# youmi-zym/TemporalStereo

Hardware: AMD Instinct MI355X
Metric: stereo pairs/sec, FlyingThings3D 540x960 D=192 (aggregation hot path) (higher is better)
Workload: dtype f32

## Files before the change

include/ts_hip.h:

```cpp
#ifndef TS_HIP_H
#define TS_HIP_H

#include <stddef.h>
#include <stdint.h>

#ifdef __cplusplus
extern "C" {
#endif

#define TS_OK 0
#define TS_ERR_NULL (-1)
#define TS_ERR_SHAPE (-2)
#define TS_ERR_UNSUPPORTED (-3)
#define TS_ERR_ALIGN (-4)

int ts_version(void);
const char* ts_last_error_string(void);

size_t ts_block_cost_workspace_bytes(int B, int C, int H, int W, int D, int scales);

int ts_block_cost_int_fwd(const float* left, const float* right, float* out, void* workspace,
                          int B, int C, int H, int W, int D, int scales, void* stream);

int ts_block_cost_sampled_fwd(const float* left, const float* right, const float* disp, float* out,
// ... 271 lines not shown
int ts_conv_wgrad_take(void* host_table, size_t capacity_bytes, int* n, int* total_blocks);
int ts_conv_wgrad_finish_many(const void* table, int n, int total_blocks, void* stream);
int ts_conv_set_chunk_cap(int cap);
int ts_conv3d_hw_fwd(const float* x, const float* w_t, const float* scale, const float* shift, float* y,
                     int B, int Cin, int Cout, int D, int H, int W, int stride, int dilation,
                     int transposed, int act, float act_param,
                     long long in_bstride, long long in_cstride, long long out_bstride,
                     long long out_cstride, const float* addend, long long addend_bstride,
                     void* workspace, size_t workspace_bytes, void* stream);
size_t ts_conv3d_hw_warp_workspace_bytes(int B, int Cout, int D, int H, int W);
int ts_conv3d_hw_warp_fwd(const float* corr, const float* w_t, const float* scale, const float* shift, float* y,
                          const float* q, const float* disp, const float* base,
                          int B, int Cc, int Cout, int D, int H, int W, int dilation, int act, float act_param,
                          long long in_bstride, long long in_cstride, long long out_bstride, long long out_cstride,
                          long long base_bstride, void* workspace, size_t workspace_bytes, void* stream);

size_t ts_conv3d_hw_workspace_bytes(int B, int Cin, int Cout, int D, int H, int W, int stride, int transposed);
int ts_conv3d_hw_x6_supported(int Cin, int Cout, int W, int stride, int dilation, int transposed);
size_t ts_conv3d_hw_x6_weight_bytes(int Cin, int Cout);
size_t ts_conv3d_hw_x6_workspace_bytes(int B, int Cin, int Cout, int D, int H, int W);
int ts_conv3d_hw_x6_weight_split(const float* w_t, void* w6, int Cin, int Cout, void* stream);
int ts_conv3d_hw_x6_weight_split_from(const float* w, void* w6, int Cin, int Cout, long long stride_ci, long long stride_co,
                                      long long stride_t, int flip, void* stream);
int ts_conv3d_hw_x6_fwd(const float* x, const void* w6, const float* scale, const float* shift, float* y,
                        int B, int Cin, int Cout, int D, int H, int W, int dilation, int act, float act_param,
                        long long in_bstride, long long in_cstride, long long out_bstride, long long out_cstride,
                        const float* addend, long long addend_bstride, void* workspace, size_t workspace_bytes, void* stream);
typedef struct ts_peer_ctx {
  void* region[8];
  int rank, world;
// ... 118 lines not shown
```

temporalstereo_amd/_lib.py:

```python
import ctypes
import os
import threading

_HERE = os.path.dirname(os.path.abspath(__file__))
LIB_PATH = os.path.join(_HERE, "libts_hip.so")

_lock = threading.Lock()
_lib = None

c_f32p = ctypes.c_void_p
c_ptr = ctypes.c_void_p
c_int = ctypes.c_int
c_size = ctypes.c_size_t
c_float = ctypes.c_float

SIGNATURES = {
    "ts_version": (c_int, []),
    "ts_last_error_string": (ctypes.c_char_p, []),
    "ts_block_cost_workspace_bytes": (c_size, [c_int] * 6),
    "ts_block_cost_int_fwd": (c_int, [c_f32p, c_f32p, c_f32p, c_ptr] + [c_int] * 6 + [c_ptr]),
    "ts_block_cost_sampled_fwd": (c_int, [c_f32p, c_f32p, c_f32p, c_f32p, c_ptr] + [c_int] * 6 + [c_ptr]),
    "ts_block_cost_sampled_warped_fwd": (c_int, [c_f32p, c_f32p, c_f32p, c_f32p, c_ptr] + [c_int] * 6 + [c_ptr]),
    "ts_block_cost_sampled_corr_fwd": (c_int, [c_f32p, c_f32p, c_f32p, c_f32p, c_ptr] + [c_int] * 6 + [c_ptr]),
    "ts_block_cost_corr_split_supported": (c_int, [c_int] * 2),
    "ts_block_cost_sampled_corr_split_fwd": (c_int, [c_f32p] * 6 + [c_ptr] + [c_int] * 7 + [ctypes.c_longlong] * 4 + [c_ptr]),
    "ts_conv3d_hw_split_supported": (c_int, [c_int] * 10),
    "ts_conv3d_hw_split_fwd": (c_int, [c_f32p] * 6 + [c_int] * 11 + [c_float] + [ctypes.c_longlong] * 6 +
                               [c_f32p, ctypes.c_longlong, c_ptr, c_size, c_ptr]),
    "ts_conv3d_d_split_supported": (c_int, [c_int] * 2),
    "ts_conv3d_d_split_fwd": (c_int, [c_f32p] * 6 + [c_int] * 13 + [c_float] + [ctypes.c_longlong] * 6 + [c_ptr]),
    "ts_conv3d_hw_x6_split_supported": (c_int, [c_int] * 5),
    "ts_conv3d_hw_x6_split_fwd": (c_int, [c_f32p, c_f32p, c_ptr, c_f32p, c_f32p, c_f32p] + [c_int] * 9 + [c_float] + [ctypes.c_longlong] * 6 +
                                  [c_f32p, ctypes.c_longlong, c_ptr, c_size, c_ptr]),
    "ts_conv3d_hw_warp_workspace_bytes": (c_size, [c_int] * 5),
    "ts_conv3d_hw_warp_fwd": (c_int, [c_f32p] * 8 + [c_int] * 8 + [c_float] + [ctypes.c_longlong] * 5 + [c_ptr, c_size, c_ptr]),
    "ts_cat_fms_fwd": (c_int, [c_f32p] * 4 + [c_int] * 5 + [c_ptr]),
    "ts_inverse_warp_3d_fwd": (c_int, [c_f32p] * 3 + [c_int] * 5 + [c_ptr]),
    "ts_dif_fms_workspace_bytes": (c_size, []),
    "ts_dif_fms_fwd": (c_int, [c_f32p] * 4 + [c_ptr] + [c_int] * 5 + [c_ptr]),
    "ts_correlation_fwd": (c_int, [c_f32p] * 3 + [c_int] * 7 + [c_ptr]),
    "ts_correlation_bwd": (c_int, [c_f32p] * 6 + [c_int] * 7 + [c_ptr]),
    "ts_block_cost_bwd_workspace_bytes": (c_size, [c_int] * 6),
    "ts_block_cost_int_bwd": (c_int, [c_f32p] * 5 + [c_ptr] + [c_int] * 6 + [c_ptr]),
    "ts_block_cost_sampled_bwd": (c_int, [c_f32p] * 7 + [c_ptr] + [c_int] * 6 + [c_ptr]),
    "ts_block_cost_sampled_warped_bwd": (c_int, [c_f32p] * 7 + [c_ptr] + [c_int] * 6 + [c_ptr]),
    "ts_calib_stream": (c_int, [c_int, c_ptr, c_ptr, c_size, c_ptr]),
    "ts_candidates_in_range_fwd": (c_int, [c_f32p] * 3 + [c_int] * 5 + [c_ptr]),
    "ts_candidates_in_range_bwd": (c_int, [c_f32p] * 5 + [c_int] * 5 + [c_ptr]),
    "ts_offset_head_fwd": (c_int, [c_f32p] * 2 + [ctypes.c_longlong, c_float, c_ptr]),
    "ts_offset_head_bwd": (c_int, [c_f32p] * 3 + [ctypes.c_longlong, c_float, c_ptr]),
# ... 122 lines not shown
    "ts_pool3d5_avgmax_bwd": (c_int, [c_f32p] * 4 + [c_int] * 5 + [c_ptr]),
    "ts_merge_candidates_bwd": (c_int, [c_f32p] * 5 + [c_int] * 5 + [c_ptr]),
    "ts_copy_rows_fwd": (c_int, [c_f32p] * 2 + [ctypes.c_longlong] * 4 + [c_ptr]),
    "ts_plan_create": (c_ptr, []),
    "ts_plan_destroy": (None, [c_ptr]),
    "ts_plan_length": (c_int, [c_ptr]),
    "ts_plan_add_call": (c_int, [c_ptr, ctypes.c_char_p, ctypes.POINTER(ctypes.c_ulonglong), c_int]),
    "ts_plan_run": (c_int, [c_ptr]),
    "ts_stream_fork": (c_int, [c_ptr, c_ptr]),
    "ts_event_record": (c_int, [c_int, c_ptr]),
    "ts_event_wait": (c_int, [c_int, c_ptr]),
}

_QUERIES = frozenset(n for n in SIGNATURES if n.endswith("_bytes") or n.startswith("ts_plan_") or
                     n.endswith("_split_supported") or
                     n in ("ts_version", "ts_last_error_string", "ts_conv_cout_pad", "ts_conv3d_hw_x6_supported", "ts_conv3d_hw_x6s_supported", "ts_peer_max_floats", "ts_peer_max_ranks",
                           "ts_peer_alloc", "ts_peer_open", "ts_peer_close", "ts_peer_free", "ts_peer_status", "ts_peer_status_async",
                           "ts_peer_set_timeout_ms", "ts_peer_reset", "ts_bn_set_small_elems",
                           "ts_conv_wgrad_defer", "ts_conv_wgrad_pending", "ts_conv_wgrad_take"))


def lib():
    rec = getattr(_tls, "recorder", None)
    if rec is not None:
        return rec.proxy
    return _real_lib()


def _real_lib():
    global _lib
    if _lib is None:
# ... 123 lines not shown
```

temporalstereo_amd/aggregation/native.py:

```python
import os
import time

import torch
import torch.nn as nn

from .. import _lib
from .. import functional as TF

ACT_NONE, ACT_SILU, ACT_RELU, ACT_TANH_OFFSET, ACT_HEAD_PAIR = 0, 1, 2, 3, 4


def _stream():
    return _lib.current_stream_handle()


_PAR = {"on": False, "aux": None, "kinds": frozenset(__import__("os").environ.get("TS_BRANCHES", "hourglass").split(","))}


def _aux_stream():
    return _PAR["aux"]


_STAGE_CAP = int(os.environ.get("TS_STAGE_CHUNK_CAP", "8"))

# ... 428 lines not shown
    rc = _lib.lib().ts_conv3d_d_fwd(_lib.ptr(x), _lib.ptr(f.w), _lib.ptr(f.scale), _lib.ptr(f.shift), _lib.ptr(out),
                                    B, Cin, f.cout, Din, H, W, k, stride, dilation, padding, int(transposed),
                                    f.act if act is None else act, float(act_param), ib, ic, ob, oc, _stream())
    _lib.check(rc, "ts_conv3d_d_fwd")
    return out


FUSED_K1 = os.environ.get("TS_FUSED_K1", "1") != "0"
SPLIT_INPUT = os.environ.get("TS_SPLIT_INPUT", "1") != "0"


def block_cost_corr(left, right, disp, scales):
    return TF.block_cost_corr(left, right, disp, scales)


def conv_hw_warp(corr, f, q, disp, base, dilation=1):
    B, Cc, D, H, W = corr.shape
    assert Cc == f.cin, (Cc, f.cin)
    out = torch.empty((B, f.cout, D, H, W), device=corr.device, dtype=torch.float32)
    ib, ic = _strides5(corr)
    ob, oc = _strides5(out)
    wsb = TF._q("ts_conv3d_hw_warp_workspace_bytes", B, f.cout, D, H, W)
    ws = torch.empty(wsb, device=corr.device, dtype=torch.uint8)
    rc = _lib.lib().ts_conv3d_hw_warp_fwd(_lib.ptr(corr), _lib.ptr(f.w), _lib.ptr(f.scale), _lib.ptr(f.shift), _lib.ptr(out),
                                          _lib.ptr(q), _lib.ptr(disp), _lib.ptr(base), B, Cc, f.cout, D, H, W, dilation, f.act, 0.0,
                                          ib, ic, ob, oc, base.stride(0) if base is not None else 0, _lib.ptr(ws), wsb, _stream())
    _lib.check(rc, "ts_conv3d_hw_warp_fwd")
    return out


def resize_add_act(a, add, size, act=ACT_SILU):
    B, C, Da, Ha, Wa = a.shape
    D, H, W = size
    out = torch.empty((B, C, D, H, W), device=a.device, dtype=torch.float32)
    ab, ac = _strides5(a)
    bb, bc = _strides5(add) if add is not None else (0, 0)
    ob, oc = _strides5(out)
    rc = _lib.lib().ts_resize3d_add_act_fwd(_lib.ptr(a), _lib.ptr(add), _lib.ptr(out), B, C, Da, Ha, Wa, D, H, W, act,
                                            ab, ac, bb, bc, ob, oc, _stream())
    _lib.check(rc, "ts_resize3d_add_act_fwd")
    return out

# ... 188 lines not shown
        self.init0, self.hg, self.init2 = SepConv(mod.init3d[0]), Hourglass(mod.init3d[1]), SepConv(mod.init3d[2])
        self.heads = Heads(mod.pred_heads)

    def init3d(self, raw, addend=None):
        return self.init2(self.hg(self.init0(raw, addend=addend)))

    def split_reference_half(self):
        if self.init0.stride != 1 or self.init0.transposed:
            raise NotImplementedError("first aggregation layer is not a stride-1 conv over [left | warped | corr]")
        self.init0_left, self.init0.f0, self.init0_corr, self.init0_q = split_sampled_first_layer(self.init0.f0, self.scales)

    def left_term(self, left):
        return conv_hw(left.unsqueeze(2), self.init0_left, 1, self.init0.dil)

    def right_term(self, right):
        return conv_d(right.unsqueeze(2), self.init0_q, 1).squeeze(2)

    def first_layer_fused(self, left, right, ds, lterm, rterm):
        corr = block_cost_corr(left, right, ds, self.scales)
        i0 = self.init0
        y = conv_hw_warp(corr, self.init0_corr, rterm, ds, lterm.squeeze(2) if lterm.dim() == 5 else lterm, i0.dil)
        return conv_d(y, i0.f1, i0.k, i0.stride, i0.dil, i0.pad_d, i0.transposed)

    def init3d_from(self, first):
        return self.init2(self.hg(first))

    def feature_terms(self, left, right):
        return self.left_term(left), (self.right_term(right) if FUSED_K1 else None)


class _MergingLevel(_LevelBase):
# ... 144 lines not shown
            return
        rc = _lib.lib().ts_deconv2d_k4s2_fwd(_lib.ptr(x), _lib.ptr(f.w), _lib.ptr(f.scale), _lib.ptr(f.shift), _lib.ptr(out),
                                             B, Cin, f.cout, H, W, f.act, out_bstride, _stream())
        _lib.check(rc, "ts_deconv2d_k4s2_fwd")

    def unet_features(self, left, right, left_image, right_image):
        both, lterm, st = self.unet_encode(left, right, left_image, right_image)
        return both, (self.unet_decode(st), lterm)

    def split_input_ok(self, B, Cf, H, W):
        L = _lib.lib()
        if self.in_planes != Cf or self.enc[3].cout != Cf:
            return False
        hw = lambda f, dil: L.ts_conv3d_hw_split_supported(B, 2 * Cf, Cf, f.cout, 1, H, W, 1, dil, 0)
        return bool(L.ts_block_cost_corr_split_supported(2 * Cf, Cf) and hw(self.init0_left, self.init0.dil) and hw(self.fuse[0], 1) and
                    (not FUSED_K1 or L.ts_conv3d_d_split_supported(2 * Cf, Cf)) and
                    (not X6 or not L.ts_conv3d_hw_x6_supported(2 * Cf, self.fuse[0].cout, W, 1, 1, 0) or
                     L.ts_conv3d_hw_x6_split_supported(2 * Cf, Cf, self.fuse[0].cout, W, 1)))

    def unet_encode(self, left, right, left_image, right_image):
        B, Cf, H, W = left.shape
        if SPLIT_INPUT and FUSED_K1 and self.split_input_ok(B, Cf, H, W):
            left, right = _lib.contiguous(left), _lib.contiguous(right)
            both = SplitBoth(left, right, torch.empty((2 * B, Cf, H, W), device=left.device, dtype=torch.float32))
            lcat, rcat = both.pair()
        else:
            both = torch.empty((2 * B, 2 * Cf, H, W), device=left.device, dtype=torch.float32)
            lcat, rcat = both[:B], both[B:]
            copy_rows(left, lcat[:, :Cf]); copy_rows(right, rcat[:, :Cf])
        C32, C2 = self.deconv4.cout, self.enc[1].cout
        cat2 = torch.empty((B, C32 + C2, 2 * H, 2 * W), device=left.device, dtype=torch.float32)
# ... 262 lines not shown
```

temporalstereo_amd/csrc/conv3d.hip:

```cpp
#include <cstdlib>
#include <mutex>
#include <type_traits>
#include <vector>

#include "conv_common.hpp"
#include "conv_x6p.hpp"
#include "warp.hpp"

namespace {




template <int MODE, int KT, int ST, int DL, int TP = 256>
struct Geom {
  static constexpr int NTR = (MODE == MODE_D) ? KT : 1;
  static constexpr int TRW = (TP == 64) ? 4 : 8, TCW = (TP == 64) ? 16 : 32;
  static constexpr int in_rows = (MODE == MODE_HW) ? (TRW - 1) * ST + 2 * DL + 1 : ((MODE == MODE_HWT) ? ((KT == 16) ? TRW + 2 : TRW + 1) : 1);
  static constexpr int in_cols = (MODE == MODE_HW) ? (TCW - 1) * ST + 2 * DL + 1 : ((MODE == MODE_HWT) ? ((KT == 16) ? TCW + 2 : TCW + 1) : TP);
  static constexpr int pitch = (MODE == MODE_D) ? TP : (in_cols | 1);
  static constexpr int RQ_HW = (in_rows * in_cols + 255) / 256;
  static constexpr int chan_raw = (MODE == MODE_D) ? NTR * TP : in_rows * pitch;
  static constexpr int pad0 = (16 - (chan_raw & 31)) & 31;
  static constexpr int chan_elems = chan_raw + (pad0 ? pad0 : 32);
// ... 1227 lines not shown
  else if (dilation == 2) rc = launch_ig<MODE_HW, 9, 1, 2>(x, w_t, scale, shift, y, p, B, tiles, D, st);
  else rc = launch_ig<MODE_HW, 9, 1, 1>(x, w_t, scale, shift, y, p, B, tiles, D, st);
  if (rc || !split) return rc;
  const long long plane = static_cast<long long>(D) * p.Ho * p.Wo;
  TS_REQUIRE(static_cast<long long>(B) * Cout <= 65535 && plane < (1ll << 31), TS_ERR_UNSUPPORTED, "conv3d_hw: split-K finish grid too large");
  long long blocks = (plane + 255) / 256;
  const long long cap = (4096 + static_cast<long long>(B) * Cout - 1) / (static_cast<long long>(B) * Cout);
  if (blocks > cap) blocks = cap;
  hipLaunchKernelGGL(conv_splitk_finish, dim3(static_cast<unsigned>(blocks), static_cast<unsigned>(B * Cout)), dim3(256), 0, st, p.partial, scale, shift, y,
                     B, Cout, plane, ksplit, act, act_param, out_bstride, out_cstride, addend, addend_bstride,
                     static_cast<long long>(p.Ho) * p.Wo);
  return ts::launched("conv_splitk_finish");
}


template <int DL>
__global__ void __launch_bounds__(256)
warp_gather_kernel(const float* __restrict__ q, const float* __restrict__ disp, const float* __restrict__ base,
                   float* __restrict__ out, int Cout, int D, int H, int W, long long base_bstride) {
  const int cogs = (Cout + 7) / 8;
  unsigned lin = blockIdx.x;
  {
    const unsigned per = gridDim.x / 8;
    if (lin < per * 8) lin = (lin % 8) * per + lin / 8;
  }
  const int d = static_cast<int>(lin % D);
  const unsigned nblk = (static_cast<unsigned>(H) * W + 255u) / 256u;
  const unsigned blk = (lin / D) % nblk;
  const int bc = static_cast<int>(lin / (static_cast<unsigned>(D) * nblk));
  const int cog = bc % cogs, b = bc / cogs;
  const unsigned HW = static_cast<unsigned>(H) * W;
// ... 8 lines not shown
#pragma unroll
  for (int t = 0; t < 9; ++t) {
    const int qy = y + (t / 3 - 1) * DL, qx = x + (t % 3 - 1) * DL;
    in[t] = live && qy >= 0 && qy < H && qx >= 0 && qx < W;
    dv[t] = __uint_as_float(__builtin_amdgcn_raw_buffer_load_b32(drs, in[t] ? (static_cast<unsigned>(qy) * W + qx) * 4u : kOOB, 0, 0));
  }
  float acc[8];
#pragma unroll
  for (int c = 0; c < 8; ++c) {
    const int co = min(cog * 8 + c, Cout - 1);
    acc[c] = (base && live) ? base[static_cast<size_t>(b) * base_bstride + static_cast<size_t>(co) * HW + pix] : 0.f;
  }
#pragma unroll
  for (int t = 0; t < 9; ++t) {
    const int qy = y + (t / 3 - 1) * DL, qx = x + (t % 3 - 1) * DL;
    const float ix = ts::source_position(qx, dv[t], W, Wm1);
    const float fl = floorf(ix);
    const float f = ix - fl;
    const int xi = static_cast<int>(fl);
    const int xb = min(max(xi, 0), W - 2);
    float wa = 0.f, wb = 0.f;
    if (xi >= 0 && xi <= W - 2) { wa = 1.f - f; wb = f; }
    else if (xi == -1) wa = f;
    else if (xi == W - 1) wb = 1.f - f;
    if (!in[t]) { wa = 0.f; wb = 0.f; }
    const unsigned voff = in[t] ? (static_cast<unsigned>(qy) * W + xb) * 4u : 0u;
#pragma unroll
    for (int c = 0; c < 8; ++c) {
      const unsigned plane = static_cast<unsigned>(t * Cout + min(cog * 8 + c, Cout - 1));
      const u32x2 v = __builtin_bit_cast(u32x2, __builtin_amdgcn_raw_buffer_load_b64(qrs, voff, plane * HW * 4u, 0));
      acc[c] += wa * __uint_as_float(v.x) + wb * __uint_as_float(v.y);
    }
  }
  if (live) {
#pragma unroll
    for (int c = 0; c < 8; ++c) {
      const int co = cog * 8 + c;
      if (co < Cout) out[((static_cast<size_t>(b) * Cout + co) * D + d) * HW + pix] = acc[c];
    }
  }
}

template <int CB, int DL, int TR = 8>
int launch_x6(const float* x, const void* w6, const float* scale, const float* shift, float* y, const IG& p, dim3 grid, hipStream_t st) {
  constexpr int NPIXP = (TR + 2 * DL) * 40;
  constexpr size_t lds = (static_cast<size_t>(3) * 2 * NPIXP + 3 * X6_SLOTS * 2 * CB * 16 + 1) * 16;
  static_assert(lds <= 80 * 1024, "ig_conv_x6_kernel: two workgroups per CU");
// ... 221 lines not shown
                                      int transposed, int act, float act_param,
                                      long long in_bstride, long long in_cstride, long long in2_bstride, long long in2_cstride,
                                      long long out_bstride, long long out_cstride, const float* addend, long long addend_bstride,
                                      void* workspace, size_t workspace_bytes, void* stream) {
  const SplitIn sp{x2, Csplit, in2_bstride, in2_cstride};
  return conv_hw_impl(x, w_t, scale, shift, y, B, Cin, Cout, D, H, W, stride, dilation, transposed, act, act_param,
                      in_bstride, in_cstride, out_bstride, out_cstride, addend, addend_bstride, workspace, workspace_bytes,
                      0, 0, stream, 0, 0, &sp);
}

extern "C" size_t ts_conv3d_hw_warp_workspace_bytes(int B, int Cout, int D, int H, int W) {
  if (B <= 0 || Cout <= 0 || D <= 0 || H <= 0 || W <= 0) return 0;
  return ts::round_up(static_cast<size_t>(B) * Cout * D * H * W * sizeof(float), 256);
}

extern "C" int ts_conv3d_hw_warp_fwd(const float* corr, const float* w_t, const float* scale, const float* shift, float* y,
                                     const float* q, const float* disp, const float* base,
                                     int B, int Cc, int Cout, int D, int H, int W, int dilation, int act, float act_param,
                                     long long in_bstride, long long in_cstride, long long out_bstride, long long out_cstride,
                                     long long base_bstride, void* workspace, size_t workspace_bytes, void* stream) {
  TS_REQUIRE(B > 0 && Cc > 0 && Cout > 0 && D > 0 && H > 0 && W >= 2, TS_ERR_SHAPE, "conv3d_hw_warp: bad size");
  TS_REQUIRE(dilation == 1 || dilation == 2, TS_ERR_UNSUPPORTED, "conv3d_hw_warp: dilation must be 1 or 2");
  TS_REQUIRE(D <= 65535 && static_cast<long long>(B) * ((Cout + 7) / 8) <= 65535, TS_ERR_UNSUPPORTED, "conv3d_hw_warp: grid too large");
  TS_REQUIRE_PTR(corr); TS_REQUIRE_PTR(w_t); TS_REQUIRE_PTR(y); TS_REQUIRE_PTR(q); TS_REQUIRE_PTR(disp); TS_REQUIRE_PTR(workspace);
  TS_REQUIRE(workspace_bytes >= ts_conv3d_hw_warp_workspace_bytes(B, Cout, D, H, W), TS_ERR_SHAPE, "conv3d_hw_warp: workspace too small");
  TS_REQUIRE(9ull * Cout * H * W * 4ull < 0x7fffffffull, TS_ERR_UNSUPPORTED, "conv3d_hw_warp: a batch element of q spans 2 GiB or more");
  hipStream_t st = ts::as_stream(stream);
  float* T = reinterpret_cast<float*>(workspace);
  const long long HW = static_cast<long long>(H) * W;
  const long long wgs = ((HW + 255) / 256) * D * B * ((Cout + 7) / 8);
  TS_REQUIRE(wgs < (1ll << 31), TS_ERR_UNSUPPORTED, "conv3d_hw_warp: grid too large");
  const dim3 grid(static_cast<unsigned>(wgs));
  if (dilation == 1) hipLaunchKernelGGL(warp_gather_kernel<1>, grid, dim3(256), 0, st, q, disp, base, T, Cout, D, H, W, base_bstride);
  else hipLaunchKernelGGL(warp_gather_kernel<2>, grid, dim3(256), 0, st, q, disp, base, T, Cout, D, H, W, base_bstride);
  if (int rc = ts::launched("warp_gather_kernel")) return rc;
  return conv_hw_impl(corr, w_t, scale, shift, y, B, Cc, Cout, D, H, W, 1, dilation, 0, act, act_param, in_bstride, in_cstride,
                      out_bstride, out_cstride, T, static_cast<long long>(Cout) * D * HW, nullptr, 0, 0, 0, stream,
                      static_cast<long long>(D) * HW, HW);
}

extern "C" int ts_conv3d_hw_bwd_data(const float* dy, const float* w_b, float* dx, int B, int Cin, int Cout, int D, int H,
                                     int W, int stride, int dilation, int transposed, long long dy_bstride,
                                     long long dy_cstride, long long dx_bstride, long long dx_cstride, void* stream) {
  TS_REQUIRE(B > 0 && Cin > 0 && Cout > 0 && D > 0 && H > 0 && W > 0, TS_ERR_SHAPE, "conv3d_hw_bwd_data: non-positive size");
  TS_REQUIRE(stride == 1 || stride == 2, TS_ERR_UNSUPPORTED, "conv3d_hw_bwd_data: stride must be 1 or 2");
  if (transposed)
    return conv_hw_impl(dy, w_b, nullptr, nullptr, dx, B, Cout, Cin, D, 2 * H, 2 * W, 2, 1, 0, ACT_NONE, 0.f, dy_bstride,
                        dy_cstride, dx_bstride, dx_cstride, nullptr, 0, nullptr, 0, 0, 0, stream);
  const int Ho = (H - 1) / stride + 1, Wo = (W - 1) / stride + 1;
  if (stride == 2)
    return conv_hw_impl(dy, w_b, nullptr, nullptr, dx, B, Cout, Cin, D, Ho, Wo, 2, 1, 1, ACT_NONE, 0.f, dy_bstride,
                        dy_cstride, dx_bstride, dx_cstride, nullptr, 0, nullptr, 0, H, W, stream);
  return conv_hw_impl(dy, w_b, nullptr, nullptr, dx, B, Cout, Cin, D, Ho, Wo, 1, dilation, 0, ACT_NONE, 0.f, dy_bstride,
// ... 228 lines not shown
```

temporalstereo_amd/csrc/plan.hip:

```cpp
#include <cstdint>
#include <cstring>
#include <mutex>
#include <string>
#include <utility>
#include <vector>

#include "ts_common.hpp"

namespace {

constexpr int kMaxWords = 32;

template <class T>
T unpack(unsigned long long w) {
  static_assert(sizeof(T) <= sizeof(unsigned long long), "argument wider than a plan word");
  T v;
  std::memcpy(&v, &w, sizeof(T));
  return v;
}

template <class... A, size_t... I>
int call_with(int (*f)(A...), const unsigned long long* w, std::index_sequence<I...>) {
  return f(unpack<A>(w[I])...);
}
// ... 57 lines not shown
    TS_PLAN_OP(ts_deconv2d_k4s2_weight_to_conv3), TS_PLAN_OP(ts_deconv2d_k4s2_wgrad_from_conv3),
    TS_PLAN_OP(ts_clip_rmsprop_step),       TS_PLAN_OP(ts_bn_sync_merge),
    TS_PLAN_OP(ts_bn_fold_many),
    TS_PLAN_OP(ts_conv_weight_layout_many2), TS_PLAN_OP(ts_conv_wgrad_finish_many), TS_PLAN_OP(ts_channel_sum_fwd),
    TS_PLAN_OP(ts_block_cost_sampled_warped_bwd),
    TS_PLAN_OP(ts_frames_prepare_fwd),      TS_PLAN_OP(ts_intrinsics_pyramid_fwd),  TS_PLAN_OP(ts_disp_u16_decode_fwd),
    TS_PLAN_OP(ts_frames_augment_fwd),      TS_PLAN_OP(ts_disp_u16_window_fwd),
    TS_PLAN_OP(ts_block_cost_sampled_corr_split_fwd), TS_PLAN_OP(ts_conv3d_hw_split_fwd),
    TS_PLAN_OP(ts_conv3d_d_split_fwd),      TS_PLAN_OP(ts_conv3d_hw_x6_split_fwd),
    TS_PLAN_OP(ts_inverse_warp_fwd),        TS_PLAN_OP(ts_inverse_warp_bwd),
    TS_PLAN_OP(ts_raft_corr_pyramid_fwd),   TS_PLAN_OP(ts_raft_corr_lookup_fwd),
    TS_PLAN_OP(ts_raft_corr_lookup_bwd),    TS_PLAN_OP(ts_raft_corr_pyramid_bwd),
    TS_PLAN_OP(ts_flow_corr_pyramid_fwd),   TS_PLAN_OP(ts_flow_corr_lookup_fwd),
    TS_PLAN_OP(ts_flow_corr_lookup_bwd),    TS_PLAN_OP(ts_flow_corr_pyramid_bwd),
    TS_PLAN_OP(ts_flow_metrics_fwd),        TS_PLAN_OP(ts_flow_render_fwd),         TS_PLAN_OP(ts_flow_u16_decode_fwd),
};

struct Call {
  const Entry* op;
  unsigned long long w[kMaxWords];
};

__global__ void __launch_bounds__(256)
copy_rows_kernel(const float* __restrict__ src, float* __restrict__ dst, long long rows, long long row_elems,
                 long long src_pitch, long long dst_pitch) {
  const long long n = rows * row_elems;
  for (long long i = static_cast<long long>(blockIdx.x) * blockDim.x + threadIdx.x; i < n;
       i += static_cast<long long>(gridDim.x) * blockDim.x) {
    const long long r = i / row_elems, c = i - r * row_elems;
    dst[r * dst_pitch + c] = src[r * src_pitch + c];
// ... 149 lines not shown
```

temporalstereo_amd/csrc/ts_common.hpp:

```cpp
#pragma once
#include <hip/hip_runtime.h>

#include <cstdarg>
#include <cstdint>
#include <cstdio>
#include <cstdlib>
#include <type_traits>

#include "../../include/ts_hip.h"

#define TS_ABI_VERSION 17

namespace ts {

char* err_buf();
int fail(int code, const char* fmt, ...);

inline hipStream_t as_stream(void* s) { return reinterpret_cast<hipStream_t>(s); }

inline bool aligned16(const void* p) { return (reinterpret_cast<uintptr_t>(p) & 15u) == 0; }

inline size_t round_up(size_t v, size_t a) { return (v + a - 1) / a * a; }

inline int launched(const char* what) {
  hipError_t e = hipGetLastError();
  if (e != hipSuccess) return fail(static_cast<int>(e), "%s: %s", what, hipGetErrorString(e));
// ... 31 lines not shown
```

Measured before the change: 1563.

## Add MFMA 1x1 conv producing tap-major q layout and vectorized warp gather

Adds a new MFMA-based 1x1 convolution kernel that writes the right-term q tensor in a channel-interleaved (groups of 8) layout, and a q8 variant of the warp gather kernel that reads 8 channels per tap with 128-bit buffer loads instead of eight strided 64-bit loads. The right_term path switches to this kernel by default when shapes allow. The aim is to cut the gather's memory transactions and replace the generic conv_d path for the pointwise projection. It adds a new layout wrapper type, so other consumers of q must handle it or call planar().

```diff
diff --git a/include/ts_hip.h b/include/ts_hip.h
--- a/include/ts_hip.h
+++ b/include/ts_hip.h
@@ -309,6 +309,15 @@
                           int B, int Cc, int Cout, int D, int H, int W, int dilation, int act, float act_param,
                           long long in_bstride, long long in_cstride, long long out_bstride, long long out_cstride,
                           long long base_bstride, void* workspace, size_t workspace_bytes, void* stream);
+int ts_conv1x1_q_supported(int Cin, int Csplit, int N);
+int ts_conv1x1_q_fwd(const float* x, const float* x2, const float* w_t, float* q, int B, int Cin, int Csplit, int N, int H, int W,
+                     long long in_bstride, long long in_cstride, long long in2_bstride, long long in2_cstride,
+                     int pixel_run, void* stream);
+int ts_conv3d_hw_warp_q8_fwd(const float* corr, const float* w_t, const float* scale, const float* shift, float* y,
+                             const float* q, const float* disp, const float* base,
+                             int B, int Cc, int Cout, int D, int H, int W, int dilation, int act, float act_param,
+                             long long in_bstride, long long in_cstride, long long out_bstride, long long out_cstride,
+                             long long base_bstride, void* workspace, size_t workspace_bytes, void* stream);
 
 size_t ts_conv3d_hw_workspace_bytes(int B, int Cin, int Cout, int D, int H, int W, int stride, int transposed);
 int ts_conv3d_hw_x6_supported(int Cin, int Cout, int W, int stride, int dilation, int transposed);
diff --git a/temporalstereo_amd/_lib.py b/temporalstereo_amd/_lib.py
--- a/temporalstereo_amd/_lib.py
+++ b/temporalstereo_amd/_lib.py
@@ -34,6 +34,9 @@
                                   [c_f32p, ctypes.c_longlong, c_ptr, c_size, c_ptr]),
     "ts_conv3d_hw_warp_workspace_bytes": (c_size, [c_int] * 5),
     "ts_conv3d_hw_warp_fwd": (c_int, [c_f32p] * 8 + [c_int] * 8 + [c_float] + [ctypes.c_longlong] * 5 + [c_ptr, c_size, c_ptr]),
+    "ts_conv3d_hw_warp_q8_fwd": (c_int, [c_f32p] * 8 + [c_int] * 8 + [c_float] + [ctypes.c_longlong] * 5 + [c_ptr, c_size, c_ptr]),
+    "ts_conv1x1_q_supported": (c_int, [c_int] * 3),
+    "ts_conv1x1_q_fwd": (c_int, [c_f32p] * 4 + [c_int] * 6 + [ctypes.c_longlong] * 4 + [c_int, c_ptr]),
     "ts_cat_fms_fwd": (c_int, [c_f32p] * 4 + [c_int] * 5 + [c_ptr]),
     "ts_inverse_warp_3d_fwd": (c_int, [c_f32p] * 3 + [c_int] * 5 + [c_ptr]),
     "ts_dif_fms_workspace_bytes": (c_size, []),
@@ -186,7 +189,7 @@
 
 _QUERIES = frozenset(n for n in SIGNATURES if n.endswith("_bytes") or n.startswith("ts_plan_") or
                      n.endswith("_split_supported") or
-                     n in ("ts_version", "ts_last_error_string", "ts_conv_cout_pad", "ts_conv3d_hw_x6_supported", "ts_conv3d_hw_x6s_supported", "ts_peer_max_floats", "ts_peer_max_ranks",
+                     n in ("ts_version", "ts_last_error_string", "ts_conv_cout_pad", "ts_conv1x1_q_supported", "ts_conv3d_hw_x6_supported", "ts_conv3d_hw_x6s_supported", "ts_peer_max_floats", "ts_peer_max_ranks",
                            "ts_peer_alloc", "ts_peer_open", "ts_peer_close", "ts_peer_free", "ts_peer_status", "ts_peer_status_async",
                            "ts_peer_set_timeout_ms", "ts_peer_reset", "ts_bn_set_small_elems",
                            "ts_conv_wgrad_defer", "ts_conv_wgrad_pending", "ts_conv_wgrad_take"))
diff --git a/temporalstereo_amd/aggregation/native.py b/temporalstereo_amd/aggregation/native.py
--- a/temporalstereo_amd/aggregation/native.py
+++ b/temporalstereo_amd/aggregation/native.py
@@ -466,6 +466,48 @@
     return TF.block_cost_corr(left, right, disp, scales)
 
 
+Q_CL = os.environ.get("TS_Q_CL", "1") != "0"
+_Q_CL_MIN_PIXELS = 4096
+
+
+class QTapMajor:
+    __slots__ = ("t",)
+
+    def __init__(self, t):
+        self.t = t
+
+    device = property(lambda self: self.t.device)
+    shape = property(lambda self: (self.t.shape[0], self.t.shape[1] * 8) + tuple(self.t.shape[2:4]))
+
+    def planar(self):
+        B, G, H, W, _ = self.t.shape
+        return self.t.permute(0, 1, 4, 2, 3).reshape(B, G * 8, H, W).contiguous()
+
+
+def conv1x1_q_ok(x, f):
+    cs = x.a.shape[1] if isinstance(x, Split) else 0
+    return bool(TF._q("ts_conv1x1_q_supported", f.cin, cs, f.cout))
+
+
+def conv1x1_q(x, f, pixel_run=0):
+    x2 = None
+    if isinstance(x, Split):
+        x, x2 = x.a, x.b
+    B, Cin, H, W = x.shape
+    cs = 0
+    i2b = i2c = 0
+    if x2 is not None:
+        cs, Cin = Cin, Cin + x2.shape[1]
+        i2b, i2c = _strides5(x2.unsqueeze(2))
+    assert Cin == f.cin and f.cout % 8 == 0, (Cin, f.cin, f.cout)
+    ib, ic = _strides5(x.unsqueeze(2))
+    out = torch.empty((B, f.cout // 8, H, W, 8), device=x.device, dtype=torch.float32)
+    rc = _lib.lib().ts_conv1x1_q_fwd(_lib.ptr(x), _lib.ptr(x2), _lib.ptr(f.w), _lib.ptr(out), B, Cin, cs, f.cout, H, W,
+                                     ib, ic, i2b, i2c, pixel_run, _stream())
+    _lib.check(rc, "ts_conv1x1_q_fwd")
+    return QTapMajor(out)
+
+
 def conv_hw_warp(corr, f, q, disp, base, dilation=1):
     B, Cc, D, H, W = corr.shape
     assert Cc == f.cin, (Cc, f.cin)
@@ -474,10 +516,13 @@
     ob, oc = _strides5(out)
     wsb = TF._q("ts_conv3d_hw_warp_workspace_bytes", B, f.cout, D, H, W)
     ws = torch.empty(wsb, device=corr.device, dtype=torch.uint8)
-    rc = _lib.lib().ts_conv3d_hw_warp_fwd(_lib.ptr(corr), _lib.ptr(f.w), _lib.ptr(f.scale), _lib.ptr(f.shift), _lib.ptr(out),
-                                          _lib.ptr(q), _lib.ptr(disp), _lib.ptr(base), B, Cc, f.cout, D, H, W, dilation, f.act, 0.0,
-                                          ib, ic, ob, oc, base.stride(0) if base is not None else 0, _lib.ptr(ws), wsb, _stream())
-    _lib.check(rc, "ts_conv3d_hw_warp_fwd")
+    name = "ts_conv3d_hw_warp_fwd"
+    if isinstance(q, QTapMajor):
+        name, q = "ts_conv3d_hw_warp_q8_fwd", q.t
+    rc = getattr(_lib.lib(), name)(_lib.ptr(corr), _lib.ptr(f.w), _lib.ptr(f.scale), _lib.ptr(f.shift), _lib.ptr(out),
+                                   _lib.ptr(q), _lib.ptr(disp), _lib.ptr(base), B, Cc, f.cout, D, H, W, dilation, f.act, 0.0,
+                                   ib, ic, ob, oc, base.stride(0) if base is not None else 0, _lib.ptr(ws), wsb, _stream())
+    _lib.check(rc, name)
     return out
 
 
@@ -696,7 +741,11 @@
         return conv_hw(left.unsqueeze(2), self.init0_left, 1, self.init0.dil)
 
     def right_term(self, right):
-        return conv_d(right.unsqueeze(2), self.init0_q, 1).squeeze(2)
+        f = self.init0_q
+        B, _, H, W = right.shape
+        if Q_CL and (f.cout // 9) % 8 == 0 and B * H * W >= _Q_CL_MIN_PIXELS and conv1x1_q_ok(right, f):
+            return conv1x1_q(right, f)
+        return conv_d(right.unsqueeze(2), f, 1).squeeze(2)
 
     def first_layer_fused(self, left, right, ds, lterm, rterm):
         corr = block_cost_corr(left, right, ds, self.scales)
@@ -871,7 +920,8 @@
             return False
         hw = lambda f, dil: L.ts_conv3d_hw_split_supported(B, 2 * Cf, Cf, f.cout, 1, H, W, 1, dil, 0)
         return bool(L.ts_block_cost_corr_split_supported(2 * Cf, Cf) and hw(self.init0_left, self.init0.dil) and hw(self.fuse[0], 1) and
-                    (not FUSED_K1 or L.ts_conv3d_d_split_supported(2 * Cf, Cf)) and
+                    (not FUSED_K1 or L.ts_conv3d_d_split_supported(2 * Cf, Cf) or
+                     (Q_CL and (self.init0_q.cout // 9) % 8 == 0 and L.ts_conv1x1_q_supported(2 * Cf, Cf, self.init0_q.cout))) and
                     (not X6 or not L.ts_conv3d_hw_x6_supported(2 * Cf, self.fuse[0].cout, W, 1, 1, 0) or
                      L.ts_conv3d_hw_x6_split_supported(2 * Cf, Cf, self.fuse[0].cout, W, 1)))
 
diff --git a/temporalstereo_amd/csrc/conv3d.hip b/temporalstereo_amd/csrc/conv3d.hip
--- a/temporalstereo_amd/csrc/conv3d.hip
+++ b/temporalstereo_amd/csrc/conv3d.hip
@@ -1265,7 +1265,24 @@
 }
 
 
-template <int DL>
+__device__ __forceinline__ void warp_tap_weights(int qx, float dv, int W, float Wm1, bool in, int& xb, float& wa, float& wb) {
+  const float ix = ts::source_position(qx, dv, W, Wm1);
+  const float fl = floorf(ix);
+  const float f = ix - fl;
+  const int xi = static_cast<int>(fl);
+  xb = min(max(xi, 0), W - 2);
+  wa = 0.f; wb = 0.f;
+  if (xi >= 0 && xi <= W - 2) { wa = 1.f - f; wb = f; }
+  else if (xi == -1) wa = f;
+  else if (xi == W - 1) wb = 1.f - f;
+  if (!in) { wa = 0.f; wb = 0.f; }
+}
+__device__ __forceinline__ void warp_tap_add(float (&acc)[8], const float (&a)[8], const float (&b)[8], float wa, float wb) {
+#pragma unroll
+  for (int c = 0; c < 8; ++c) acc[c] += wa * a[c] + wb * b[c];
+}
+
+template <int DL, bool Q8>
 __global__ void __launch_bounds__(256)
 warp_gather_kernel(const float* __restrict__ q, const float* __restrict__ disp, const float* __restrict__ base,
                    float* __restrict__ out, int Cout, int D, int H, int W, long long base_bstride) {
@@ -1304,23 +1321,33 @@
 #pragma unroll
   for (int t = 0; t < 9; ++t) {
     const int qy = y + (t / 3 - 1) * DL, qx = x + (t % 3 - 1) * DL;
-    const float ix = ts::source_position(qx, dv[t], W, Wm1);
-    const float fl = floorf(ix);
-    const float f = ix - fl;
-    const int xi = static_cast<int>(fl);
-    const int xb = min(max(xi, 0), W - 2);
-    float wa = 0.f, wb = 0.f;
-    if (xi >= 0 && xi <= W - 2) { wa = 1.f - f; wb = f; }
-    else if (xi == -1) wa = f;
-    else if (xi == W - 1) wb = 1.f - f;
-    if (!in[t]) { wa = 0.f; wb = 0.f; }
-    const unsigned voff = in[t] ? (static_cast<unsigned>(qy) * W + xb) * 4u : 0u;
-#pragma unroll
-    for (int c = 0; c < 8; ++c) {
-      const unsigned plane = static_cast<unsigned>(t * Cout + min(cog * 8 + c, Cout - 1));
-      const u32x2 v = __builtin_bit_cast(u32x2, __builtin_amdgcn_raw_buffer_load_b64(qrs, voff, plane * HW * 4u, 0));
-      acc[c] += wa * __uint_as_float(v.x) + wb * __uint_as_float(v.y);
-    }
+    int xb;
+    float wa, wb;
+    warp_tap_weights(qx, dv[t], W, Wm1, in[t], xb, wa, wb);
+    float va[8], vb[8];
+    if constexpr (Q8) {
+      const unsigned voff = in[t] ? (static_cast<unsigned>(qy) * W + xb) * 32u : 0u;
+      const unsigned plane = static_cast<unsigned>(t * cogs + cog);
+      u32x4 v[4];
+#pragma unroll
+      for (int i = 0; i < 4; ++i) v[i] = __builtin_amdgcn_raw_buffer_load_b128(qrs, voff + i * 16u, plane * HW * 32u, 0);
+#pragma unroll
+      for (int i = 0; i < 2; ++i) {
+        va[4 * i + 0] = __uint_as_float(v[i].x); va[4 * i + 1] = __uint_as_float(v[i].y);
+        va[4 * i + 2] = __uint_as_float(v[i].z); va[4 * i + 3] = __uint_as_float(v[i].w);
+        vb[4 * i + 0] = __uint_as_float(v[2 + i].x); vb[4 * i + 1] = __uint_as_float(v[2 + i].y);
+        vb[4 * i + 2] = __uint_as_float(v[2 + i].z); vb[4 * i + 3] = __uint_as_float(v[2 + i].w);
+      }
+    } else {
+      const unsigned voff = in[t] ? (static_cast<unsigned>(qy) * W + xb) * 4u : 0u;
+#pragma unroll
+      for (int c = 0; c < 8; ++c) {
+        const unsigned plane = static_cast<unsigned>(t * Cout + min(cog * 8 + c, Cout - 1));
+        const u32x2 v = __builtin_bit_cast(u32x2, __builtin_amdgcn_raw_buffer_load_b64(qrs, voff, plane * HW * 4u, 0));
+        va[c] = __uint_as_float(v.x); vb[c] = __uint_as_float(v.y);
+      }
+    }
+    warp_tap_add(acc, va, vb, wa, wb);
   }
   if (live) {
 #pragma unroll
@@ -1572,29 +1599,56 @@
   return ts::round_up(static_cast<size_t>(B) * Cout * D * H * W * sizeof(float), 256);
 }
 
-extern "C" int ts_conv3d_hw_warp_fwd(const float* corr, const float* w_t, const float* scale, const float* shift, float* y,
-                                     const float* q, const float* disp, const float* base,
-                                     int B, int Cc, int Cout, int D, int H, int W, int dilation, int act, float act_param,
-                                     long long in_bstride, long long in_cstride, long long out_bstride, long long out_cstride,
-                                     long long base_bstride, void* workspace, size_t workspace_bytes, void* stream) {
+namespace {
+int conv_hw_warp_impl(const float* corr, const float* w_t, const float* scale, const float* shift, float* y,
+                      const float* q, const float* disp, const float* base,
+                      int B, int Cc, int Cout, int D, int H, int W, int dilation, int act, float act_param,
+                      long long in_bstride, long long in_cstride, long long out_bstride, long long out_cstride,
+                      long long base_bstride, void* workspace, size_t workspace_bytes, void* stream, bool q8) {
   TS_REQUIRE(B > 0 && Cc > 0 && Cout > 0 && D > 0 && H > 0 && W >= 2, TS_ERR_SHAPE, "conv3d_hw_warp: bad size");
   TS_REQUIRE(dilation == 1 || dilation == 2, TS_ERR_UNSUPPORTED, "conv3d_hw_warp: dilation must be 1 or 2");
+  TS_REQUIRE(!q8 || Cout % 8 == 0, TS_ERR_UNSUPPORTED, "conv3d_hw_warp_q8: Cout=%d is not a multiple of 8", Cout);
   TS_REQUIRE(D <= 65535 && static_cast<long long>(B) * ((Cout + 7) / 8) <= 65535, TS_ERR_UNSUPPORTED, "conv3d_hw_warp: grid too large");
   TS_REQUIRE_PTR(corr); TS_REQUIRE_PTR(w_t); TS_REQUIRE_PTR(y); TS_REQUIRE_PTR(q); TS_REQUIRE_PTR(disp); TS_REQUIRE_PTR(workspace);
   TS_REQUIRE(workspace_bytes >= ts_conv3d_hw_warp_workspace_bytes(B, Cout, D, H, W), TS_ERR_SHAPE, "conv3d_hw_warp: workspace too small");
   TS_REQUIRE(9ull * Cout * H * W * 4ull < 0x7fffffffull, TS_ERR_UNSUPPORTED, "conv3d_hw_warp: a batch element of q spans 2 GiB or more");
+  if (q8) TS_REQUIRE_ALIGNED(q);
   hipStream_t st = ts::as_stream(stream);
   float* T = reinterpret_cast<float*>(workspace);
   const long long HW = static_cast<long long>(H) * W;
   const long long wgs = ((HW + 255) / 256) * D * B * ((Cout + 7) / 8);
   TS_REQUIRE(wgs < (1ll << 31), TS_ERR_UNSUPPORTED, "conv3d_hw_warp: grid too large");
   const dim3 grid(static_cast<unsigned>(wgs));
-  if (dilation == 1) hipLaunchKernelGGL(warp_gather_kernel<1>, grid, dim3(256), 0, st, q, disp, base, T, Cout, D, H, W, base_bstride);
-  else hipLaunchKernelGGL(warp_gather_kernel<2>, grid, dim3(256), 0, st, q, disp, base, T, Cout, D, H, W, base_bstride);
+  if (q8) {
+    if (dilation == 1) hipLaunchKernelGGL((warp_gather_kernel<1, true>), grid, dim3(256), 0, st, q, disp, base, T, Cout, D, H, W, base_bstride);
+    else hipLaunchKernelGGL((warp_gather_kernel<2, true>), grid, dim3(256), 0, st, q, disp, base, T, Cout, D, H, W, base_bstride);
+  } else {
+    if (dilation == 1) hipLaunchKernelGGL((warp_gather_kernel<1, false>), grid, dim3(256), 0, st, q, disp, base, T, Cout, D, H, W, base_bstride);
+    else hipLaunchKernelGGL((warp_gather_kernel<2, false>), grid, dim3(256), 0, st, q, disp, base, T, Cout, D, H, W, base_bstride);
+  }
   if (int rc = ts::launched("warp_gather_kernel")) return rc;
   return conv_hw_impl(corr, w_t, scale, shift, y, B, Cc, Cout, D, H, W, 1, dilation, 0, act, act_param, in_bstride, in_cstride,
                       out_bstride, out_cstride, T, static_cast<long long>(Cout) * D * HW, nullptr, 0, 0, 0, stream,
                       static_cast<long long>(D) * HW, HW);
+}
+}
+
+extern "C" int ts_conv3d_hw_warp_fwd(const float* corr, const float* w_t, const float* scale, const float* shift, float* y,
+                                     const float* q, const float* disp, const float* base,
+                                     int B, int Cc, int Cout, int D, int H, int W, int dilation, int act, float act_param,
+                                     long long in_bstride, long long in_cstride, long long out_bstride, long long out_cstride,
+                                     long long base_bstride, void* workspace, size_t workspace_bytes, void* stream) {
+  return conv_hw_warp_impl(corr, w_t, scale, shift, y, q, disp, base, B, Cc, Cout, D, H, W, dilation, act, act_param, in_bstride, in_cstride,
+                           out_bstride, out_cstride, base_bstride, workspace, workspace_bytes, stream, false);
+}
+
+extern "C" int ts_conv3d_hw_warp_q8_fwd(const float* corr, const float* w_t, const float* scale, const float* shift, float* y,
+                                        const float* q, const float* disp, const float* base,
+                                        int B, int Cc, int Cout, int D, int H, int W, int dilation, int act, float act_param,
+                                        long long in_bstride, long long in_cstride, long long out_bstride, long long out_cstride,
+                                        long long base_bstride, void* workspace, size_t workspace_bytes, void* stream) {
+  return conv_hw_warp_impl(corr, w_t, scale, shift, y, q, disp, base, B, Cc, Cout, D, H, W, dilation, act, act_param, in_bstride, in_cstride,
+                           out_bstride, out_cstride, base_bstride, workspace, workspace_bytes, stream, true);
 }
 
 extern "C" int ts_conv3d_hw_bwd_data(const float* dy, const float* w_b, float* dx, int B, int Cin, int Cout, int D, int H,
diff --git a/temporalstereo_amd/csrc/conv_pw.hip b/temporalstereo_amd/csrc/conv_pw.hip
--- /dev/null
+++ b/temporalstereo_amd/csrc/conv_pw.hip
@@ -0,0 +1,228 @@
+#include "conv_common.hpp"
+
+namespace {
+
+struct PW {
+  const float* x;
+  const float* x2;
+  const float* w;
+  float* q;
+  int Cin, csplit, N, pad;
+  unsigned HW;
+  long long bs1, cs1, bs2, cs2;
+  unsigned in_bytes, in2_bytes, w_bytes, q_bytes;
+};
+
+constexpr int PW_KC = 32;
+constexpr size_t PW_LDS = 160 * 1024;
+
+__host__ __device__ constexpr int pw_wpitch(int mtg) { return mtg * 16 + (mtg % 2 == 0 ? 16 : 0); }
+
+template <int PR, int MTW, bool VEC>
+__global__ void __launch_bounds__(256)
+conv_pw_kernel(const PW p) {
+  constexpr int WP = PR / 32, WM = 4 / WP;
+  constexpr int CAP = MTW * WM;
+  constexpr int WS = pw_wpitch(CAP);
+  constexpr int XS = PR + 16;
+  constexpr int QPR = PR / 4;
+  constexpr int NL = PW_KC * QPR / 256;
+  constexpr int RING = PR == 128 ? 2 : 4;
+  extern __shared__ float4 pw_smem[];
+  float* const ws = reinterpret_cast<float*>(pw_smem);
+  float* const xs = ws + static_cast<size_t>(p.Cin) * WS;
+
+  const int tid = threadIdx.x, lane = tid & 63, wave = __builtin_amdgcn_readfirstlane(tid >> 6);
+  const int wp = wave % WP, wm = wave / WP;
+  const int b = blockIdx.z;
+  const unsigned pix0 = blockIdx.x * static_cast<unsigned>(PR);
+  const int tiles_all = (p.N + 15) / 16;
+  const int t0 = blockIdx.y * CAP;
+  const int mtiles = min(CAP, tiles_all - t0);
+  const int n0 = t0 * 16;
+  const int nch = (p.Cin + PW_KC - 1) / PW_KC;
+
+  const __amdgpu_buffer_rsrc_t r1 = ig_rsrc(p.x + static_cast<size_t>(b) * p.bs1, p.in_bytes);
+  const __amdgpu_buffer_rsrc_t r2 = p.x2 ? ig_rsrc(p.x2 + static_cast<size_t>(b) * p.bs2, p.in2_bytes) : r1;
+  const unsigned cs1b = static_cast<unsigned>(p.cs1) * 4u, cs2b = static_cast<unsigned>(p.cs2) * 4u;
+
+  u32x4 ring[RING][NL];
+  auto load_chunk = [&](int ch, u32x4 (&r)[NL]) {
+    const int c0 = ch * PW_KC;
+    const ChunkBase cb = chunk_base(c0, p.csplit, r1, r2, cs1b, cs2b);
+#pragma unroll
+    for (int i = 0; i < NL; ++i) {
+      const int idx = i * 256 + tid, row = idx / QPR, piece = idx % QPR;
+      const unsigned px = pix0 + piece * 4u;
+      const bool ok = c0 + row < p.Cin;
+      const unsigned off = static_cast<unsigned>(c0 + row - cb.c_first) * cb.cstride_b + px * 4u;
+      if constexpr (VEC) {
+        r[i] = __builtin_amdgcn_raw_buffer_load_b128(cb.rsrc, (ok && px < p.HW) ? off : kOOB, 0, 0);
+      } else {
+        r[i].x = __builtin_amdgcn_raw_buffer_load_b32(cb.rsrc, (ok && px + 0u < p.HW) ? off : kOOB, 0, 0);
+        r[i].y = __builtin_amdgcn_raw_buffer_load_b32(cb.rsrc, (ok && px + 1u < p.HW) ? off + 4u : kOOB, 0, 0);
+        r[i].z = __builtin_amdgcn_raw_buffer_load_b32(cb.rsrc, (ok && px + 2u < p.HW) ? off + 8u : kOOB, 0, 0);
+        r[i].w = __builtin_amdgcn_raw_buffer_load_b32(cb.rsrc, (ok && px + 3u < p.HW) ? off + 12u : kOOB, 0, 0);
+      }
+    }
+  };
+  auto store_chunk = [&](int buf, const u32x4 (&r)[NL]) {
+#pragma unroll
+    for (int i = 0; i < NL; ++i) {
+      const int idx = i * 256 + tid, row = idx / QPR, piece = idx % QPR;
+      *reinterpret_cast<u32x4*>(xs + (buf * PW_KC + row) * XS + piece * 4) = r[i];
+    }
+  };
+
+#pragma unroll
+  for (int s = 0; s < RING; ++s)
+    if (s < nch) load_chunk(s, ring[s]);
+  {
+    const __amdgpu_buffer_rsrc_t wr = ig_rsrc(p.w, p.w_bytes);
+    constexpr int qrow = CAP * 4;
+    const int total = p.Cin * qrow;
+    constexpr int WB = 6;
+    for (int first = tid; first < total; first += 256 * WB) {
+      u32x4 v[WB];
+#pragma unroll
+      for (int i = 0; i < WB; ++i) {
+        const int idx = first + i * 256, c = idx / qrow, j = idx - c * qrow;
+        const int n = n0 + j * 4;
+        v[i] = __builtin_amdgcn_raw_buffer_load_b128(wr, (idx < total && j < mtiles * 4 && n < p.pad) ? static_cast<unsigned>(c * p.pad + n) * 4u : kOOB, 0, 0);
+      }
+#pragma unroll
+      for (int i = 0; i < WB; ++i) {
+        const int idx = first + i * 256, c = idx / qrow, j = idx - c * qrow;
+        if (idx < total) *reinterpret_cast<u32x4*>(ws + c * WS + j * 4) = v[i];
+      }
+    }
+  }
+
+  v4f acc[MTW][2];
+#pragma unroll
+  for (int j = 0; j < MTW; ++j) { acc[j][0] = v4f{0.f, 0.f, 0.f, 0.f}; acc[j][1] = v4f{0.f, 0.f, 0.f, 0.f}; }
+
+  const int lrow = lane >> 4, lcol = lane & 15;
+  for (int ch0 = 0; ch0 < nch; ch0 += RING) {
+#pragma unroll
+    for (int s = 0; s < RING; ++s) {
+      const int ch = ch0 + s;
+      if (ch < nch) {
+        const int buf = s & 1;
+        store_chunk(buf, ring[s]);
+        if (ch + RING < nch) load_chunk(ch + RING, ring[s]);
+        __syncthreads();
+        const int c0 = ch * PW_KC;
+        const int ksteps = min(PW_KC, p.Cin - c0) / 4;
+        const float* xb = xs + (buf * PW_KC + lrow) * XS + wp * 32 + lcol;
+        const float* wb = ws + (c0 + lrow) * WS + wm * 16 + lcol;
+        float a[MTW], b0, b1;
+        auto operands = [&](int ks, float (&ra)[MTW], float& rb0, float& rb1) {
+          rb0 = xb[ks * 4 * XS]; rb1 = xb[ks * 4 * XS + 16];
+#pragma unroll
+          for (int j = 0; j < MTW; ++j) ra[j] = wb[ks * 4 * WS + j * WM * 16];
+        };
+        auto products = [&](const float (&ra)[MTW], float rb0, float rb1) {
+#pragma unroll
+          for (int j = 0; j < MTW; ++j) {
+            acc[j][0] = __builtin_amdgcn_mfma_f32_16x16x4f32(ra[j], rb0, acc[j][0], 0, 0, 0);
+            acc[j][1] = __builtin_amdgcn_mfma_f32_16x16x4f32(ra[j], rb1, acc[j][1], 0, 0, 0);
+          }
+        };
+        operands(0, a, b0, b1);
+        for (int ks = 0; ks < ksteps; ks += 2) {
+          float an[MTW], bn0, bn1;
+          operands(ks + 1, an, bn0, bn1);
+          __builtin_amdgcn_sched_barrier(0);
+          products(a, b0, b1);
+          __builtin_amdgcn_sched_barrier(0);
+          operands(min(ks + 2, ksteps - 1), a, b0, b1);
+          __builtin_amdgcn_sched_barrier(0);
+          products(an, bn0, bn1);
+          __builtin_amdgcn_sched_barrier(0);
+        }
+      }
+    }
+  }
+
+  const __amdgpu_buffer_rsrc_t qr = ig_rsrc(p.q + static_cast<size_t>(b) * p.N * p.HW, p.q_bytes);
+#pragma unroll
+  for (int j = 0; j < MTW; ++j) {
+    const int n = n0 + (wm + j * WM) * 16 + lrow * 4;
+#pragma unroll
+    for (int pt = 0; pt < 2; ++pt) {
+      const unsigned px = pix0 + wp * 32 + pt * 16 + lcol;
+      const unsigned off = ((static_cast<unsigned>(n >> 3) * p.HW + px) * 8u + static_cast<unsigned>(n & 7)) * 4u;
+      __builtin_amdgcn_raw_buffer_store_b128(__builtin_bit_cast(u32x4, acc[j][pt]), qr, (n < p.N && px < p.HW) ? off : kOOB, 0, 0);
+    }
+  }
+}
+
+bool pw_split_ok(int Cin, int Csplit) { return Csplit > 0 && Csplit < Cin && Csplit % 32 == 0; }
+
+size_t pw_lds_bytes(int Cin, int PR, int cap) { return (static_cast<size_t>(Cin) * pw_wpitch(cap) + static_cast<size_t>(2) * PW_KC * (PR + 16)) * 4; }
+
+template <int PR, int MTW, bool VEC>
+int pw_launch(const PW& p, int B, hipStream_t st) {
+  constexpr int CAP = MTW * (4 / (PR / 32));
+  const size_t lds = pw_lds_bytes(p.Cin, PR, CAP);
+  const int groups = ((p.N + 15) / 16 + CAP - 1) / CAP;
+  const unsigned long long runs = (static_cast<unsigned long long>(p.HW) + PR - 1) / PR;
+  TS_REQUIRE(lds <= PW_LDS && groups <= 65535 && B <= 65535, TS_ERR_UNSUPPORTED, "conv1x1_q: grid too large");
+  auto kern = &conv_pw_kernel<PR, MTW, VEC>;
+  if (lds > 64 * 1024)
+    (void)hipFuncSetAttribute(reinterpret_cast<const void*>(kern), hipFuncAttributeMaxDynamicSharedMemorySize, static_cast<int>(lds));
+  hipLaunchKernelGGL(kern, dim3(static_cast<unsigned>(runs), static_cast<unsigned>(groups), static_cast<unsigned>(B)), dim3(256), lds, st, p);
+  return ts::launched("conv_pw_kernel");
+}
+
+template <int PR, bool VEC>
+int pw_launch_run(const PW& p, int B, hipStream_t st) {
+  constexpr int WM = 4 / (PR / 32), NARROW = PR == 128 ? 5 : 2, WIDE = PR == 128 ? 9 : 3;
+  if ((p.N + 15) / 16 > NARROW * WM && pw_lds_bytes(p.Cin, PR, WIDE * WM) <= PW_LDS) return pw_launch<PR, WIDE, VEC>(p, B, st);
+  return pw_launch<PR, NARROW, VEC>(p, B, st);
+}
+
+}
+
+extern "C" int ts_conv1x1_q_supported(int Cin, int Csplit, int N) {
+  if (Cin <= 0 || N <= 0 || Cin % 8 != 0 || N % 8 != 0) return 0;
+  if (Csplit != 0 && !pw_split_ok(Cin, Csplit)) return 0;
+  return pw_lds_bytes(Cin, 128, 5) <= PW_LDS && pw_lds_bytes(Cin, 32, 8) <= PW_LDS;
+}
+
+extern "C" int ts_conv1x1_q_fwd(const float* x, const float* x2, const float* w_t, float* q, int B, int Cin, int Csplit, int N, int H, int W,
+                                long long in_bstride, long long in_cstride, long long in2_bstride, long long in2_cstride,
+                                int pixel_run, void* stream) {
+  TS_REQUIRE(B > 0 && Cin > 0 && N > 0 && H > 0 && W > 0, TS_ERR_SHAPE, "conv1x1_q: non-positive size");
+  TS_REQUIRE(pixel_run == 0 || pixel_run == 32 || pixel_run == 128, TS_ERR_SHAPE, "conv1x1_q: pixel_run %d is not 0, 32 or 128", pixel_run);
+  TS_REQUIRE_PTR(x); TS_REQUIRE_PTR(w_t); TS_REQUIRE_PTR(q);
+  TS_REQUIRE(x2 != nullptr || Csplit == 0, TS_ERR_NULL, "conv1x1_q: Csplit=%d without x2", Csplit);
+  TS_REQUIRE(ts_conv1x1_q_supported(Cin, x2 ? Csplit : 0, N) && (!x2 || pw_split_ok(Cin, Csplit)), TS_ERR_UNSUPPORTED,
+             "conv1x1_q: Cin=%d (multiple of 8, at most 256), Csplit=%d (multiple of 32 inside (0, Cin)), N=%d (multiple of 8)", Cin, Csplit, N);
+  TS_REQUIRE_ALIGNED(w_t); TS_REQUIRE_ALIGNED(q);
+  const int pad = ts_conv_cout_pad(N);
+  const unsigned long long HW = static_cast<unsigned long long>(H) * W;
+  const int c1 = x2 ? Csplit : Cin;
+  TS_REQUIRE(in_cstride >= 0 && in2_cstride >= 0, TS_ERR_UNSUPPORTED, "conv1x1_q: negative channel stride");
+  const unsigned long long b1 = (static_cast<unsigned long long>(c1 - 1) * in_cstride + HW) * 4ull;
+  const unsigned long long b2 = x2 ? (static_cast<unsigned long long>(Cin - Csplit - 1) * in2_cstride + HW) * 4ull : 0ull;
+  const unsigned long long wb = static_cast<unsigned long long>(Cin) * pad * 4ull, qb = static_cast<unsigned long long>(N) * HW * 4ull;
+  TS_REQUIRE(b1 < 0x7fffffffull && b2 < 0x7fffffffull && wb < 0x7fffffffull && qb < 0x7fffffffull, TS_ERR_UNSUPPORTED,
+             "conv1x1_q: a batch element of x, x2 or q, or the weight array, spans 2 GiB or more");
+  int PR = pixel_run;
+  if (PR == 0)
+    PR = static_cast<long long>((HW + 127) / 128) * B >= ts::kNumCU * 3 / 4 ? 128 : 32;
+  PW p;
+  p.x = x; p.x2 = x2; p.w = w_t; p.q = q;
+  p.Cin = Cin; p.csplit = x2 ? Csplit : 0x7fffffff; p.N = N; p.pad = pad;
+  p.HW = static_cast<unsigned>(HW);
+  p.bs1 = in_bstride; p.cs1 = in_cstride; p.bs2 = x2 ? in2_bstride : 0; p.cs2 = x2 ? in2_cstride : 0;
+  p.in_bytes = static_cast<unsigned>(b1); p.in2_bytes = static_cast<unsigned>(b2);
+  p.w_bytes = static_cast<unsigned>(wb); p.q_bytes = static_cast<unsigned>(qb);
+  hipStream_t st = ts::as_stream(stream);
+  auto quads = [&](const float* ptr, long long bs, long long cs) { return ts::aligned16(ptr) && bs % 4 == 0 && cs % 4 == 0; };
+  const bool vec = HW % 4 == 0 && quads(x, in_bstride, in_cstride) && (!x2 || quads(x2, in2_bstride, in2_cstride));
+  if (PR == 128) return vec ? pw_launch_run<128, true>(p, B, st) : pw_launch_run<128, false>(p, B, st);
+  return vec ? pw_launch_run<32, true>(p, B, st) : pw_launch_run<32, false>(p, B, st);
+}
diff --git a/temporalstereo_amd/csrc/plan.hip b/temporalstereo_amd/csrc/plan.hip
--- a/temporalstereo_amd/csrc/plan.hip
+++ b/temporalstereo_amd/csrc/plan.hip
@@ -95,6 +95,7 @@
     TS_PLAN_OP(ts_flow_corr_pyramid_fwd),   TS_PLAN_OP(ts_flow_corr_lookup_fwd),
     TS_PLAN_OP(ts_flow_corr_lookup_bwd),    TS_PLAN_OP(ts_flow_corr_pyramid_bwd),
     TS_PLAN_OP(ts_flow_metrics_fwd),        TS_PLAN_OP(ts_flow_render_fwd),         TS_PLAN_OP(ts_flow_u16_decode_fwd),
+    TS_PLAN_OP(ts_conv1x1_q_fwd),           TS_PLAN_OP(ts_conv3d_hw_warp_q8_fwd),
 };
 
 struct Call {
diff --git a/temporalstereo_amd/csrc/ts_common.hpp b/temporalstereo_amd/csrc/ts_common.hpp
--- a/temporalstereo_amd/csrc/ts_common.hpp
+++ b/temporalstereo_amd/csrc/ts_common.hpp
@@ -9,7 +9,7 @@
 
 #include "../../include/ts_hip.h"
 
-#define TS_ABI_VERSION 17
+#define TS_ABI_VERSION 18
 
 namespace ts {
 
```

Result: no change. 1576 (median of 4 runs) (+0.8%).
